# sMedX/FaceNet

Hardware: AMD Instinct MI355X
Metric: images/sec (160x160 triplet train) (higher is better)
Workload: dtype bf16

## Files before the change

facenet_amd/_lib.py:

```python
from __future__ import annotations

import ctypes as C
import os

import torch

_HERE = os.path.dirname(os.path.abspath(__file__))
LIB_PATH = os.path.join(_HERE, "lib", "libfacenet_hip.so")

FN_BF16, FN_F16 = 0, 1


class ConvDesc(C.Structure):
    _fields_ = [
        ("N", C.c_int32), ("H", C.c_int32), ("W", C.c_int32), ("Cin", C.c_int32),
        ("OH", C.c_int32), ("OW", C.c_int32), ("Cout", C.c_int32),
        ("KH", C.c_int32), ("KW", C.c_int32), ("stride", C.c_int32), ("pad_h", C.c_int32), ("pad_w", C.c_int32),
        ("dtype", C.c_int32), ("ld_x", C.c_int32), ("ld_y", C.c_int32),
        ("relu", C.c_int32), ("accumulate", C.c_int32), ("out_f32", C.c_int32), ("ld_res", C.c_int32),
        ("scale", C.c_float), ("splits", C.c_int32), ("stats_sq_off", C.c_int32), ("stats_replicas", C.c_int32),
        ("stats_rep_stride", C.c_int32),
        ("x", C.c_void_p), ("w", C.c_void_p), ("y", C.c_void_p), ("dx", C.c_void_p), ("dw", C.c_void_p),
        ("bias", C.c_void_p), ("stats", C.c_void_p), ("resid", C.c_void_p),
        ("bn_y", C.c_void_p), ("bn_scale", C.c_void_p), ("bn_shift", C.c_void_p), ("bn_beta", C.c_void_p), ("bn_acc", C.c_void_p),
        ("ld_bn_y", C.c_int32), ("bn_sq_off", C.c_int32), ("bn_replicas", C.c_int32), ("bn_rep_stride", C.c_int32), ("bn_relu", C.c_int32),
        ("nrm_stats", C.c_void_p), ("nrm_beta", C.c_void_p),
        ("nrm_sq_off", C.c_int32), ("nrm_replicas", C.c_int32), ("nrm_rep_stride", C.c_int32), ("nrm_count", C.c_int32),
        ("nrm_eps", C.c_float), ("nrm_z", C.c_void_p), ("tile_fwd", C.c_int32), ("tile_dgrad", C.c_int32),
        ("dy2", C.c_void_p), ("w2", C.c_void_p), ("dy3", C.c_void_p), ("w3", C.c_void_p),
        ("Cout2", C.c_int32), ("ld_y2", C.c_int32), ("Cout3", C.c_int32), ("ld_y3", C.c_int32),
        ("rb_prev", C.c_void_p), ("rb_out", C.c_void_p), ("rb_dtrunk", C.c_void_p), ("rb_dup", C.c_void_p), ("rb_dbias", C.c_void_p),
        ("rb_scale", C.c_float), ("rb_accumulate", C.c_int32), ("prelu", C.c_void_p),
    ]


class FacenetHipError(RuntimeError):
    pass


_i, _f, _p, _l, _u = C.c_int, C.c_float, C.c_void_p, C.c_long, C.c_uint32

_SIGNATURES = {
    "fn_abi_version": [],
    "fn_conv2d_fwd": [C.POINTER(ConvDesc), _p],
    "fn_conv2d_dgrad": [C.POINTER(ConvDesc), _p],
    "fn_conv2d_wgrad": [C.POINTER(ConvDesc), _p],
    "fn_conv2d_variant": [C.POINTER(ConvDesc), _i],
    "fn_block35_infer": [_p, _p, _i, _p, _p, _p, _p, _p, _p, _f, _i, _i, _p],
    "fn_block35_infer_warm": [_p, _p, _i, _p, _p, _p, _p, _p, _p, _f, _i, _p, C.c_int64, _i, _p],
    "fn_block17_infer": [_p, _p, _i, _p, _p, _p, _p, _p, _p, _p, _p, _p, _p, _f, _i, _i, _p],
    "fn_block17_infer_warm": [_p, _p, _i, _p, _p, _p, _p, _p, _p, _p, _p, _p, _p, _f, _i, _p, C.c_int64, _i, _p],
    "fn_conv2d_arg_bytes": [],
    "fn_conv2d_group_build": [C.POINTER(ConvDesc), _i, _i, _i, _p, _p, _p],
    "fn_conv2d_grouped": [_p, _p, _i, _i, _i, _i, _i, _i, _p],
    "fn_conv2d_wgrad_arg_bytes": [],
    "fn_conv2d_wgrad_group_build": [C.POINTER(ConvDesc), _i, _i, _p, _p, _p, _p],
    "fn_conv2d_wgrad_reduce": [_p, _i, _p],
    "fn_conv2d_wgrad_grouped": [_p, _p, _i, _i, _i, _i, _p],
    "fn_image_normalize": [_p, _p, _p, _i, _i, _i, _i, _p],
    "fn_image_normalize_f32": [_p, _p, _p, _i, _i, _i, _i, _p],
    "fn_image_resize_bilinear": [_p, _i, _p, _i, _i, _i, _i, _i, _p],
    "fn_bn_finalize": [_p, _i, _i, _p, _p, _p, _p, _p, _p, _p, _f, _f, _i, _p],
    "fn_crop_or_pad_u8": [_p, _p, _p, _p, _i, _i, _p],
    "fn_gather_images": [_p, _p, _p, _i, _i, _p],
    "fn_bn_relu_train_fwd": [_p, _i, _p, _i, _i, _i, _p, _i, _i, _i, _p, _p, _p, _p, _p, _f, _f, _i, _i, _p],
    "fn_bn_relu_train_bwd": [_p, _i, _p, _i, _i, _i, _p, _p, _p, _p, _p, _i, _i, _i, _i, _i, _i, _p],
    "fn_maxpool3x3s2_fwd": [_p, _i, _p, _i, _i, _i, _i, _i, _p, _i, _p],
    "fn_maxpool3x3s2_bwd": [_p, _i, _p, _i, _p, _i, _i, _i, _i, _i, _p, _i, _i, _p],
    "fn_area_resize_crop": [_p, _i, _i, _p, _i, _i, _i, _i, _p, _i, _p],
    "fn_maxpool2d_fwd": [_p, _i, _p, _i, _i, _i, _i, _i, _i, _i, _i, _i, _i, _i, _i, _p],
    "fn_area_resize_frame": [_p, _i, _i, _i, _i, _p, _p, _i, _p],
    "fn_mtcnn_candidates": [_p, C.c_long, _i, _f, _p, _p, _i, _i, _i, _p],
    "fn_nms_greedy_batch": [_p, _i, _p, _p, _p, _p, _i, _p, C.c_long, _p, _p, _p],
    "fn_nms_greedy": [_p, _i, _p, _i, C.c_double, _i, _p, C.c_long, _p, _p, _p],
    "fn_avgpool_fwd": [_p, _p, _i, _i, _i, _i, _p],
    "fn_avgpool_bwd": [_p, _p, _i, _i, _i, _i, _p],
    "fn_avgpool3x3s1_fwd": [_p, _i, _p, _i, _i, _i, _i, _i, _i, _p],
    "fn_avgpool3x3s1_bwd": [_p, _i, _p, _i, _i, _i, _i, _i, _i, _i, _p],
    "fn_dropout_fwd": [_p, _p, _i, _i, _f, _u, _i, _p, _i, _p],
    "fn_dropout_bwd": [_p, _p, _i, _i, _f, _u, _i, _p, _i, _p],
# ... 61 lines not shown
```

facenet_amd/csrc/conv_igemm.hip:

```cpp
#include "common.h"
#include "../../include/facenet_hip.h"
#include "wgrad_taps.h"
#include <cstdio>
#include <type_traits>
#include <cstdlib>

#ifndef FN_IG_DBG
#define FN_IG_DBG 0
#endif

#if FN_IG_DBG & 32
__device__ unsigned long long fn_ig_phase[256 * 576 * 16];
extern "C" int fn_debug_phases(unsigned long long* out, int reset) {
    static unsigned long long host[256 * 576 * 16];
    if (out) {
        if (hipMemcpyFromSymbol(host, HIP_SYMBOL(fn_ig_phase), sizeof(host)) != hipSuccess) return -1;
        for (int i = 0; i < 576 * 16; ++i) {
            out[i] = 0;
            for (int r = 0; r < 256; ++r) out[i] += host[r * 576 * 16 + i];
        }
    }
    if (reset) {
        for (auto& v : host) v = 0;
        if (hipMemcpyToSymbol(HIP_SYMBOL(fn_ig_phase), host, sizeof(host)) != hipSuccess) return -1;
// ... 22 lines not shown
    const unsigned short* resid;
    int M, PH, PW;
    int SH, SW;
    int CS;
    int NOUT, KTOT, KH, KW;
    int so, sk, offy, offx, dshift;
    int ld_src, ld_out, ld_res;
    int relu, accumulate, out_f32;
    float scale;
    int tiles_m, tiles_n;
    int stats_sq_off, stats_replicas, stats_rep_stride;
    int plain;
    const unsigned short* bn_y;
    const float* bn_scale;
    const float* bn_shift;
    const float* bn_beta;
    acc_t* bn_acc;
    int ld_bn_y, bn_sq_off, bn_replicas, bn_rep_stride, bn_relu;
    int s2;
    int cp1, cp2, cp3;
    int total_tiles;
    int src_bytes, w_bytes;
    int tile;
    int nocheck;
    const unsigned short* src2; const unsigned short* wp2;
    const unsigned short* src3; const unsigned short* wp3;
    int K2, ld2, K3, ld3, t1, t2, nt_total, src2_bytes, w2_bytes, src3_bytes, w3_bytes;
    const acc_t* nrm_stats;
    const float* nrm_beta;
    int nrm_sq_off, nrm_replicas, nrm_rep_stride, nrm_count;
    float nrm_eps;
    unsigned short* nrm_z;
    int halo_ty, halo_tx;
    const unsigned short* mask;
    unsigned short* out2;
    acc_t* colsum;
    float scale2;
    const float* prelu;
};

__device__ __forceinline__ void rcp_divmod(int m, int d, int& q, int& r) { fast_divmod(m, d, __builtin_amdgcn_rcpf((float)d), q, r); }

__device__ __forceinline__ int ktab_entry_s2(int kgroup, int CS, int KH, int KW, int qy, int qx) {
    const int nky = (KH - qy + 1) >> 1, nkx = (KW - qx + 1) >> 1;
    const int k = kgroup * 8;
    if (k >= nky * nkx * CS) return -1;
    int tap, c, ty, tx;
    rcp_divmod(k, CS, tap, c);
    rcp_divmod(tap, nkx, ty, tx);
    return ((qy + 2 * ty) << 24) | ((qx + 2 * tx) << 16) | c;
}

__device__ __forceinline__ int ktab_entry(int kgroup, int KTOT, int CS, int KW) {
    const int k = kgroup * 8;
    if (k >= KTOT) return -1;
    int tap, c, ky, kx;
    rcp_divmod(k, CS, tap, c);
    rcp_divmod(tap, KW, ky, kx);
    return (ky << 24) | (kx << 16) | c;
}

template <typename T, int BM, int BN, int WM, int WN, bool MULTI = false>
__device__ __forceinline__ void conv_epilogue(const ConvArgs& a, f32x4 (&acc)[BM / WM / 16][BN / WN / 16], unsigned char* smem, float* sRed,
                                              const int* sRow, const bool rowtab, const int m0, const int n0, const int tm, const bool active FN_EP_PARAM) {
    constexpr int TM = BM / WM, TN = BN / WN;
    constexpr int MREP = TM / 16, NREP = TN / 16;
// ... 887 lines not shown
enum { TILE_HALO = 9000000 };
static bool halo_capable(const ConvArgs& a) {
    return !a.s2 && !a.plain && a.so == 1 && a.dshift == 0 && a.KH == 3 && a.KW == 3 && a.CS % 8 == 0 && !a.nrm_stats && a.nt_total == 0;
}
static bool halo_eligible(const ConvArgs& a) {
    if (a.tile == TILE_HALO) return halo_capable(a);
    static const int enabled = getenv("FN_CONV_HALO") ? atoi(getenv("FN_CONV_HALO")) : 1;
    static const int maxc = getenv("FN_CONV_HALO_MAXC") ? atoi(getenv("FN_CONV_HALO_MAXC")) : 64;
    return enabled && halo_capable(a) && a.CS <= maxc && a.PH >= 30 && a.PW >= 30 &&
           a.tile == 0;
}
static int halo_bn(const ConvArgs& a) { return a.NOUT <= 32 ? 32 : (a.NOUT <= 48 || (a.NOUT > 64 && a.NOUT <= 96) ? 32 : 64); }

template <typename T, int BN, int WM, int WN, int KH, int KW> static int launch_halo_p(ConvArgs a, hipStream_t st) {
    a.halo_ty = cdiv(a.PH, 8);
    a.halo_tx = cdiv(a.PW, 16);
    a.tiles_n = cdiv(a.NOUT, BN);
    a.tiles_m = 0;
    const long total = (long)(a.M / (a.PH * a.PW)) * a.halo_ty * a.halo_tx * a.tiles_n;
    FN_REQUIRE(total < (1L << 24), "conv_halo: too many tiles");
    a.total_tiles = (int)total;
    const size_t smem = halo_smem_bytes(BN, KH, KW);
    auto kern = conv_halo_kernel<T, BN, WM, WN, KH, KW>;
    static LdsOptIn lds_ok;
    if (int rc = allow_big_lds(reinterpret_cast<const void*>(kern), lds_ok, "conv_halo")) return rc;
    hipLaunchKernelGGL(kern, dim3(a.total_tiles), dim3(256), smem, st, a);
    return check_launch("conv_halo");
}

template <typename T> static int launch_halo(const ConvArgs& a, hipStream_t st) {
    return halo_bn(a) == 32 ? launch_halo_p<T, 32, 4, 1, 3, 3>(a, st) : launch_halo_p<T, 64, 2, 2, 3, 3>(a, st);
}

static void plan_tiles(ConvArgs& a, int BM, int BN) {
    a.tiles_n = cdiv(a.NOUT, BN);
    if (!a.s2) {
        a.tiles_m = cdiv(a.M, BM);
        a.total_tiles = a.tiles_m * a.tiles_n;
        return;
    }
    const int nimg = a.M / (a.PH * a.PW);
    int ny[4], nx[4], pre[5];
    int t = 0;
    for (int c = 0; c < 4; ++c) {
        const int qy = c >> 1, qx = c & 1;
        const int y0 = (qy - a.offy) & 1, x0 = (qx - a.offx) & 1;
        ny[c] = a.PH > y0 ? (a.PH - y0 + 1) / 2 : 0;
        nx[c] = a.PW > x0 ? (a.PW - x0 + 1) / 2 : 0;
        pre[c] = t;
        t += cdiv(nimg * ny[c] * nx[c], BM) * a.tiles_n;
    }
    a.cp1 = pre[1]; a.cp2 = pre[2]; a.cp3 = pre[3];
    a.tiles_m = 0;
    a.total_tiles = t;
}

static size_t conv_smem_bytes(int BM, int BN, int KTOT, int plain, int norm_channels, int ks) {
    const int STAGE = ks * 2 * (BM * 128 + BN * 128);
    const int CB = BM * (BN + 4) * 4;
    return (size_t)(STAGE > CB ? STAGE : CB) + 8 * BN * 4 + (plain ? 0 : (size_t)cdiv(KTOT, 64) * 8 * 16) + (size_t)BM * 4 +
           (size_t)norm_channels * 8;
}

template <typename T, int BM, int BN, int WM, int WN, int DEPTH, int KS, bool PLAIN, int MODE>
static int launch_conv_grouped_p(const ConvArgs* dev_args, const int32_t* dev_prefix, int n, int total, size_t smem, hipStream_t st) {
    auto kern = conv_igemm_grouped_kernel<T, BM, BN, WM, WN, DEPTH, KS, PLAIN, MODE>;
// ... 20 lines not shown
}

template <typename T, int BM, int BN, int WM, int WN, int DEPTH, int KS>
static int launch_conv(const ConvArgs& a, hipStream_t st) {
    if constexpr (KS == 1) {
        if (a.nt_total > 0) return launch_conv_p<T, BM, BN, WM, WN, DEPTH, 1, true, 2>(a, st);
        if (a.nrm_stats)
            return a.plain ? launch_conv_p<T, BM, BN, WM, WN, DEPTH, 1, true, 1>(a, st) : launch_conv_p<T, BM, BN, WM, WN, DEPTH, 1, false, 1>(a, st);
    }
    return a.plain ? launch_conv_p<T, BM, BN, WM, WN, DEPTH, KS, true, 0>(a, st) : launch_conv_p<T, BM, BN, WM, WN, DEPTH, KS, false, 0>(a, st);
}

static void choose_conv_tile_auto(int M, int NOUT, int& bm, int& bn) {
    bn = 128;
    long best = (long)cdiv(NOUT, 128) * 128;
    for (int c : {64, 32}) {
        const long w = (long)cdiv(NOUT, c) * c;
        if (w < best) { best = w; bn = c; }
    }
    static const int minb = getenv("FN_CONV_MINBLOCKS") ? atoi(getenv("FN_CONV_MINBLOCKS")) : 384;
    bm = 32;
    for (int c : {128, 64}) {
        if ((long)cdiv(M, c) * cdiv(NOUT, bn) >= minb) { bm = c; break; }
    }
    while (bm == 32 && bn > 32 && (long)cdiv(M, 32) * cdiv(NOUT, bn) < minb) bn >>= 1;
}

static void choose_conv_tile(int M, int NOUT, int forced, int& bm, int& bn) {
    if (forced > 0) { bm = forced / 1000; bn = forced % 1000; return; }
    choose_conv_tile_auto(M, NOUT, bm, bn);
}

static bool valid_tile(int t) {
    if (t == 0 || t == TILE_HALO) return true;
    const int bm = t / 1000, bn = t % 1000;
    return (bm == 128 || bm == 64 || bm == 32) && (bn == 128 || bn == 64 || bn == 32);
}

static int choose_conv_ks(int M, int NOUT, int KTOT, int bm, int bn) {
    static const int force = getenv("FN_CONV_KS") ? atoi(getenv("FN_CONV_KS")) : 0;
    if (bm == 64) {
        static const int ks64 = getenv("FN_CONV_KS64") ? atoi(getenv("FN_CONV_KS64")) : 256;
        static const int ks64_4 = getenv("FN_CONV_KS64_4") ? atoi(getenv("FN_CONV_KS64_4")) : 0;
        const long grid = (long)cdiv(M, 64) * cdiv(NOUT, bn);
        if (force != 1 && force != 2 && bn <= 64 && cdiv(KTOT, 64) >= 12 && grid <= ks64_4) return 4;
        return (force != 1 && bn <= 64 && cdiv(KTOT, 64) >= 8 && grid <= ks64) ? 2 : 1;
    }
    if (bm != 32) return 1;
    const long blocks = (long)cdiv(M, 32) * cdiv(NOUT, bn);
    const int ntk = cdiv(KTOT, 64);
    static const int lim2 = getenv("FN_CONV_KS32_2") ? atoi(getenv("FN_CONV_KS32_2")) : 128;
    static const int lim4 = getenv("FN_CONV_KS32_4") ? atoi(getenv("FN_CONV_KS32_4")) : 64;
    int ks = 1;
    if (ntk >= 8 && blocks <= lim2) ks = 2;
    if (ntk >= 16 && blocks <= lim4 && bn <= 64) ks = 4;
    if (force == 1) ks = 1;
    if (force == 2 && ks > 2) ks = 2;
    return ks;
}

#define FN_CONV_VARIANTS(X) X(128, 128, 2, 2, 1, 1) X(128, 64, 2, 2, 2, 1) X(128, 32, 4, 1, 2, 1) X(64, 128, 1, 4, 2, 1) X(64, 64, 2, 2, 2, 1) \
    X(64, 32, 2, 2, 2, 1) X(32, 128, 1, 4, 4, 1) X(32, 64, 1, 4, 4, 1) X(32, 32, 2, 2, 4, 1)                                           \
    X(32, 128, 1, 4, 4, 2) X(32, 64, 1, 4, 4, 2) X(32, 64, 1, 4, 4, 4) X(32, 32, 2, 2, 4, 2) X(32, 32, 2, 2, 4, 4)                       \
    X(64, 64, 2, 2, 2, 2) X(64, 32, 2, 2, 2, 2) X(64, 64, 2, 2, 2, 4) X(64, 32, 2, 2, 2, 4)

static int variant_code(int bm, int bn, int ks) { return bm * 1000 + bn + (ks > 1 ? ks * 1000000 : 0); }

template <typename T> static int dispatch_conv(const ConvArgs& a, hipStream_t st) {
    if (halo_eligible(a)) return launch_halo<T>(a, st);
    if (a.tile == TILE_HALO) {
        set_error("conv: the halo-tile kernel was requested (tile %d) for a layer it cannot run (needs 3x3, stride 1, channels %% 8 == 0)", a.tile);
        return FN_EUNSUPPORTED;
    }
    int bm, bn;
    choose_conv_tile(a.M, a.NOUT, a.tile, bm, bn);
    if (const char* f = getenv("FN_CONV_TILE")) {
        int fm = 0, fnn = 0;
        if (sscanf(f, "%dx%d", &fm, &fnn) == 2) { bm = fm; bn = fnn; }
    }
    const int ks = (a.nrm_stats || a.nt_total > 0) ? 1 : choose_conv_ks(a.M, a.NOUT, a.KTOT, bm, bn);
#define FN_X(BM_, BN_, WM_, WN_, D_, KS_) \
    if (bm == BM_ && bn == BN_ && ks == KS_) return launch_conv<T, BM_, BN_, WM_, WN_, D_, KS_>(a, st);
    FN_CONV_VARIANTS(FN_X)
#undef FN_X
    set_error("conv: no tile variant %dx%d ks=%d", bm, bn, ks);
    return FN_EUNSUPPORTED;
}

template <typename T>
static int dispatch_conv_grouped(const ConvArgs* dev_args, const int32_t* dev_prefix, int n, int total, int bm, int bn, int ks, int plain,
                                 size_t smem, hipStream_t st) {
    const bool norm = (plain & 2) != 0;
    plain &= 1;
#define FN_X(BM_, BN_, WM_, WN_, D_, KS_)                                                                                                       \
    if (bm == BM_ && bn == BN_ && ks == KS_) {                                                                                                  \
        if constexpr (KS_ == 1) {                                                                                                               \
            if (norm)                                                                                                                           \
                return plain ? launch_conv_grouped_p<T, BM_, BN_, WM_, WN_, D_, 1, true, 1>(dev_args, dev_prefix, n, total, smem, st)         \
                             : launch_conv_grouped_p<T, BM_, BN_, WM_, WN_, D_, 1, false, 1>(dev_args, dev_prefix, n, total, smem, st);       \
        }                                                                                                                                       \
        return plain ? launch_conv_grouped_p<T, BM_, BN_, WM_, WN_, D_, KS_, true, 0>(dev_args, dev_prefix, n, total, smem, st)              \
// ... 346 lines not shown
    return bnw == 64 ? launch_wgrad<T, 128, 64>(a, splits, st) : launch_wgrad<T, 128, 128>(a, splits, st);
}

}

using namespace fn;

static int make_fwd_args(const fn_conv_desc* d, ConvArgs& a) {
    if (int rc = check_desc(d)) return rc;
    FN_REQUIRE(d->x && d->w && d->y, "conv_fwd: null x/w/y");
    FN_REQUIRE(d->ld_y >= d->Cout && (d->out_f32 ? d->ld_y % 4 == 0 : d->ld_y % 8 == 0), "conv_fwd: ld_y=%d invalid", d->ld_y);
    FN_REQUIRE(!d->resid || d->ld_res % 8 == 0, "conv_fwd: ld_res=%d invalid", d->ld_res);
    a = ConvArgs{};
    a.src = (const unsigned short*)d->x; a.wp = (const unsigned short*)d->w; a.out = d->y;
    a.bias = d->bias; a.stats = d->stats; a.resid = (const unsigned short*)d->resid;
    FN_REQUIRE(!d->prelu || (!d->resid && !d->relu && !d->accumulate && !d->stats), "conv_fwd: prelu excludes resid / relu / accumulate / stats");
    a.prelu = d->prelu;
    a.M = d->N * d->OH * d->OW; a.PH = d->OH; a.PW = d->OW; a.SH = d->H; a.SW = d->W; a.CS = d->Cin;
    a.NOUT = d->Cout; a.KTOT = d->KH * d->KW * d->Cin; a.KH = d->KH; a.KW = d->KW;
    a.so = d->stride; a.sk = 1; a.offy = -d->pad_h; a.offx = -d->pad_w; a.dshift = 0;
    a.ld_src = d->ld_x; a.ld_out = d->ld_y; a.ld_res = d->ld_res;
    a.relu = d->relu; a.accumulate = d->accumulate; a.out_f32 = d->out_f32; a.scale = d->scale;
    a.stats_sq_off = d->stats_sq_off;
    a.plain = (d->KH == 1 && d->KW == 1 && d->stride == 1 && d->pad_h == 0 && d->pad_w == 0) ? 1 : 0;
    a.nocheck = (d->pad_h == 0 && d->pad_w == 0) ? 1 : 0;
    a.stats_replicas = d->stats_replicas > 0 ? d->stats_replicas : 1;
    a.stats_rep_stride = d->stats_rep_stride;
    FN_REQUIRE((long)d->N * d->H * d->W * d->ld_x * 2 < (1L << 30) && (long)d->Cout * a.KTOT * 2 < (1L << 30),
               "conv_fwd: x or w exceeds the 1 GiB range of 32-bit buffer offsets");
    FN_REQUIRE((long)a.M * d->ld_y * (d->out_f32 ? 4 : 2) < (1L << 31) && (!d->resid || (long)a.M * d->ld_res * 2 < (1L << 31)),
               "conv_fwd: y or the residual exceeds the 2 GiB range of 32-bit byte offsets");
    a.src_bytes = d->N * d->H * d->W * d->ld_x * 2;
    a.w_bytes = d->Cout * a.KTOT * 2;
    FN_REQUIRE(valid_tile(d->tile_fwd), "conv_fwd: tile_fwd=%d is not one of {128,64,32}x{128,64,32} or 9000000 (halo)", d->tile_fwd);
    a.tile = d->tile_fwd;
    if (d->nrm_stats) {
        FN_REQUIRE(d->nrm_beta && d->Cin <= 512 && d->nrm_count > 0 && d->nrm_eps > 0.f, "conv_fwd: normalise-on-load needs beta, Cin <= 512, count, eps");
        a.nrm_stats = d->nrm_stats; a.nrm_beta = d->nrm_beta; a.nrm_sq_off = d->nrm_sq_off;
        a.nrm_replicas = d->nrm_replicas > 0 ? d->nrm_replicas : 1; a.nrm_rep_stride = d->nrm_rep_stride;
        a.nrm_count = d->nrm_count; a.nrm_eps = d->nrm_eps;
        if (d->nrm_z) {
            FN_REQUIRE(d->stride == 1 && d->OH == d->H && d->OW == d->W, "conv_fwd: nrm_z needs stride 1 and an output map of the input's size");
            a.nrm_z = (unsigned short*)d->nrm_z;
        }
    } else {
        FN_REQUIRE(!d->nrm_z, "conv_fwd: nrm_z without nrm_stats");
    }
    return FN_OK;
}

static int make_dgrad_args(const fn_conv_desc* d, ConvArgs& a) {
    if (int rc = check_desc(d)) return rc;
    FN_REQUIRE(d->y && d->w && (d->dx || d->rb_dup), "conv_dgrad: null dy/wt/dx");
    FN_REQUIRE(d->Cout % 8 == 0 && d->ld_y % 8 == 0 && d->ld_y >= d->Cout, "conv_dgrad: Cout=%d ld_y=%d must be multiples of 8", d->Cout,
               d->ld_y);
    a = ConvArgs{};
    a.src = (const unsigned short*)d->y; a.wp = (const unsigned short*)d->w; a.out = d->dx;
    a.M = d->N * d->H * d->W; a.PH = d->H; a.PW = d->W; a.SH = d->OH; a.SW = d->OW; a.CS = d->Cout;
    a.NOUT = d->Cin; a.KTOT = d->KH * d->KW * d->Cout; a.KH = d->KH; a.KW = d->KW;
    a.so = 1; a.sk = -1; a.offy = d->pad_h; a.offx = d->pad_w; a.dshift = d->stride == 2 ? 1 : 0;
    a.s2 = d->stride == 2 ? 1 : 0;
    a.ld_src = d->ld_y; a.ld_out = d->ld_x; a.ld_res = 0;
    a.relu = 0; a.accumulate = d->accumulate; a.out_f32 = d->out_f32; a.scale = 1.f;
    a.plain = (d->KH == 1 && d->KW == 1 && d->stride == 1 && d->pad_h == 0 && d->pad_w == 0) ? 1 : 0;
    a.stats_replicas = 1;
    FN_REQUIRE((long)d->N * d->OH * d->OW * d->ld_y * 2 < (1L << 30) && (long)d->Cin * a.KTOT * 2 < (1L << 30),
               "conv_dgrad: dy or wt exceeds the 1 GiB range of 32-bit buffer offsets");
    FN_REQUIRE((long)d->N * d->H * d->W * d->ld_x * (d->out_f32 ? 4 : 2) < (1L << 31) &&
                   (!d->bn_y || (long)d->N * d->H * d->W * d->ld_bn_y * 2 < (1L << 31)),
               "conv_dgrad: dx or bn_y exceeds the 2 GiB range of 32-bit byte offsets");
    a.src_bytes = d->N * d->OH * d->OW * d->ld_y * 2;
    a.w_bytes = d->Cin * a.KTOT * 2;
    FN_REQUIRE(valid_tile(d->tile_dgrad), "conv_dgrad: tile_dgrad=%d is not one of {128,64,32}x{128,64,32} or 9000000 (halo)", d->tile_dgrad);
    a.tile = d->tile_dgrad;
    if (d->dy2) {
        FN_REQUIRE(a.plain && d->w2 && d->Cout2 > 0 && d->Cout2 % 8 == 0 && d->ld_y2 % 8 == 0 && d->ld_y2 >= d->Cout2 && !d->bn_y,
                   "conv_dgrad: sibling sources need a 1x1 stride-1 layer, w2 and Cout2/ld_y2 multiples of 8");
        FN_REQUIRE(!d->dy3 || (d->w3 && d->Cout3 > 0 && d->Cout3 % 8 == 0 && d->ld_y3 % 8 == 0 && d->ld_y3 >= d->Cout3),
                   "conv_dgrad: third source needs w3 and Cout3/ld_y3 multiples of 8");
        const long pix = (long)d->N * d->OH * d->OW;
        FN_REQUIRE(pix * d->ld_y2 * 2 < (1L << 30) && (!d->dy3 || pix * d->ld_y3 * 2 < (1L << 30)), "conv_dgrad: sibling dy exceeds 1 GiB");
        a.src2 = (const unsigned short*)d->dy2; a.wp2 = (const unsigned short*)d->w2; a.K2 = d->Cout2; a.ld2 = d->ld_y2;
        a.src2_bytes = (int)(pix * d->ld_y2 * 2); a.w2_bytes = d->Cin * d->Cout2 * 2;
        a.t1 = cdiv(a.KTOT, 64);
        a.t2 = a.t1 + cdiv(a.K2, 64);
        a.nt_total = a.t2;
        if (d->dy3) {
            a.src3 = (const unsigned short*)d->dy3; a.wp3 = (const unsigned short*)d->w3; a.K3 = d->Cout3; a.ld3 = d->ld_y3;
            a.src3_bytes = (int)(pix * d->ld_y3 * 2); a.w3_bytes = d->Cin * d->Cout3 * 2;
            a.nt_total = a.t2 + cdiv(a.K3, 64);
        }
    }
    if (d->rb_dup) {
        FN_REQUIRE(d->rb_dtrunk && d->rb_dbias && !d->bn_y && !d->out_f32 && d->Cin % 8 == 0 && d->ld_x % 8 == 0,
                   "conv_dgrad: fused residual backward needs rb_dtrunk, rb_dbias, a low-precision dx geometry and no fused BN reduction");
        a.out = d->rb_dtrunk; a.accumulate = d->rb_accumulate;
        a.resid = (const unsigned short*)d->rb_prev; a.ld_res = d->ld_x; a.scale = 1.f;
        a.mask = (const unsigned short*)d->rb_out; a.out2 = (unsigned short*)d->rb_dup; a.colsum = d->rb_dbias; a.scale2 = d->rb_scale;
    }
    if (d->bn_y) {
        FN_REQUIRE(!d->accumulate && !d->out_f32 && d->bn_scale && d->bn_shift && d->bn_beta && d->bn_acc && d->ld_bn_y % 8 == 0,
                   "conv_dgrad: fused BN reduction needs a sole-writer low-precision dx and all bn_* pointers");
        a.bn_y = (const unsigned short*)d->bn_y; a.bn_scale = d->bn_scale; a.bn_shift = d->bn_shift; a.bn_beta = d->bn_beta;
        a.bn_acc = d->bn_acc; a.ld_bn_y = d->ld_bn_y; a.bn_sq_off = d->bn_sq_off;
        a.bn_replicas = d->bn_replicas > 0 ? d->bn_replicas : 1; a.bn_rep_stride = d->bn_rep_stride; a.bn_relu = d->bn_relu;
    }
// ... 154 lines not shown
}

template <typename T> static int launch_wgrad_grouped(const void* args, const int32_t* prefix, int n, int total, int variant, hipStream_t st) {
    const bool norm = variant >= 1000000;
    variant %= 1000000;
    const int bmw = variant / 1000, bnw = variant % 1000;
    const unsigned char* a = reinterpret_cast<const unsigned char*>(args);
    const int stride_ = fn_conv2d_wgrad_arg_bytes();
#define FN_WG(BM_, BN_)                                                                                                     \
    if (bmw == BM_ && bnw == BN_) {                                                                                         \
        const size_t sm_ = 2 * 64 * ((BM_) * 2 + 32 + (BN_) * 2 + 32) + (norm ? 2 * (BN_) * 4 : 0);                            \
        if (norm) hipLaunchKernelGGL((conv_wgrad_grouped_kernel<T, BM_, BN_, true>), dim3(total), dim3(256), sm_, st, a, stride_, prefix, n); \
        else hipLaunchKernelGGL((conv_wgrad_grouped_kernel<T, BM_, BN_, false>), dim3(total), dim3(256), sm_, st, a, stride_, prefix, n);    \
        return check_launch("conv_wgrad_grouped");                                                                          \
    }
    FN_WG(32, 64) FN_WG(32, 128) FN_WG(64, 64) FN_WG(64, 128) FN_WG(128, 64) FN_WG(128, 128)
#undef FN_WG
    set_error("wgrad_grouped: unknown variant %d", variant);
    return FN_EINVAL;
}

extern "C" int fn_conv2d_wgrad_grouped(const void* dev_args, const int32_t* dev_prefix, int n, int total_blocks, int variant, int dtype,
                                       void* stream) {
    FN_REQUIRE(dev_args && dev_prefix && n > 0 && total_blocks > 0, "wgrad_grouped: bad arguments");
    FN_REQUIRE(dtype == FN_BF16 || dtype == FN_F16, "dtype %d unsupported", dtype);
    if (variant >= WGRAD_TAPS_VARIANT) return wgrad_taps_launch(dev_args, dev_prefix, n, total_blocks, variant, dtype, (hipStream_t)stream);
    return dtype == FN_BF16 ? launch_wgrad_grouped<__bf16>(dev_args, dev_prefix, n, total_blocks, variant, (hipStream_t)stream)
                            : launch_wgrad_grouped<_Float16>(dev_args, dev_prefix, n, total_blocks, variant, (hipStream_t)stream);
}

extern "C" int fn_conv2d_variant(const fn_conv_desc* d, int op) {
    if (!d || op < 0 || op > 2) return FN_EINVAL;
    int a, b;
    if (op < 2) {
        ConvArgs ca;
        if ((op == 0 ? make_fwd_args(d, ca) : make_dgrad_args(d, ca)) == FN_OK && halo_eligible(ca)) return 9000000 + halo_bn(ca);
        if ((op == 0 ? d->tile_fwd : d->tile_dgrad) == TILE_HALO) return FN_EUNSUPPORTED;
    }
    if (op == 0) {
        choose_conv_tile(d->N * d->OH * d->OW, d->Cout, valid_tile(d->tile_fwd) ? d->tile_fwd : 0, a, b);
        return variant_code(a, b, d->nrm_stats ? 1 : choose_conv_ks(d->N * d->OH * d->OW, d->Cout, d->KH * d->KW * d->Cin, a, b));
    }
    if (op == 1) {
        choose_conv_tile(d->N * d->H * d->W, d->Cin, valid_tile(d->tile_dgrad) ? d->tile_dgrad : 0, a, b);
        return variant_code(a, b, d->dy2 ? 1 : choose_conv_ks(d->N * d->H * d->W, d->Cin, d->KH * d->KW * d->Cout, a, b));
    }
    if (const int tv = wgrad_taps_variant(d)) return tv;
    final_wgrad_tile(d->Cout, d->KH * d->KW * d->Cin, a, b);
    return a * 1000 + b;
}
```

facenet_amd/train.py:

```python
from __future__ import annotations

import ctypes as C
import json
import os
from typing import Callable, Dict, List, Optional, Sequence, Tuple

import numpy as np
import torch

from . import _lib, parallel
from .engine import BN_EPS, L2_WEIGHT, Lowering, Network, _pad8, _ptr
from .schedule import Op, Schedule, StreamSet, levelize, make_events, region, run_schedule, torch_op


class GraphRunner:

    def __init__(self, device: torch.device):
        self.device = device
        self.graphs: List[torch.cuda.CUDAGraph] = []
        self.pool = None

    def capture(self, fn: Callable[[], None]) -> torch.cuda.CUDAGraph:
        g = torch.cuda.CUDAGraph()
        with torch.cuda.graph(g, pool=self.pool):
# ... 27 lines not shown
        total = lib.fn_conv2d_wgrad_group_build(descs, n, variant, host_args, host_prefix, None, C.byref(ws_elems))
        if total < 0:
            _lib.check(total, "wgrad_group_build")
        ws = torch.empty(max(1, ws_elems.value), dtype=torch.float32, device=net.device)
        total = lib.fn_conv2d_wgrad_group_build(descs, n, variant, host_args, host_prefix, _ptr(ws), C.byref(ws_elems))
        if total < 0:
            _lib.check(total, "wgrad_group_build")
        dev_args = torch.frombuffer(bytearray(host_args), dtype=torch.uint8).to(net.device)
        dev_prefix = torch.tensor(list(host_prefix), dtype=torch.int32, device=net.device)
        reads, writes = [], []
        for m in members:
            reads.extend(m.reads)
            writes.extend(m.writes)
        if variant >= 5000000:
            code = variant - 5000000
            name = f"conv_wgrad_taps:{code // 1000}x{code % 1000 // 10}" + ("s2" if code % 10 else "")
        else:
            name = f"conv_wgrad_grouped:{variant % 1000000 // 1000}x{variant % 1000}" + (":norm" if variant >= 1000000 else "")
        out.append(Op(name, lib.fn_conv2d_wgrad_grouped,
                      (_ptr(dev_args), _ptr(dev_prefix), n, total, variant, dt), keep=(descs, dev_args, dev_prefix, members, ws),
                      reads=tuple(reads), writes=tuple(writes) + (region(ws),)))
        if ws_elems.value > 0:
            split_tables.append(dev_args)
            split_keep.append(ws)
            split_writes.extend(writes)
    if split_tables:
        table = torch.cat(split_tables)
        out.append(Op("conv_wgrad_reduce", lib.fn_conv2d_wgrad_reduce, (_ptr(table), table.numel() // nbytes), keep=(table, split_keep),
                      reads=tuple(region(w) for w in split_keep), writes=tuple(split_writes)))
    return out


TILE_CANDIDATES = tuple((bm, bn) for bm in (128, 64, 32) for bn in (128, 64, 32))


def autotune_convs(ops: Sequence[Op], net: Network, launches: int = 8, rounds: int = 2) -> Dict[str, int]:
    if os.environ.get("FACENET_AUTOTUNE", "1") == "0":
        return {}
    lib, st = net.lib, net.stream()
    chosen: Dict[str, int] = {}
    cache_path = os.environ.get("FACENET_TUNE_CACHE")
    cache: Dict[str, int] = {}
    if cache_path and os.path.exists(cache_path):
        with open(cache_path) as fh:
            cache = json.load(fh)
    dirty = False

    def burst(op):
        a, b = torch.cuda.Event(enable_timing=True), torch.cuda.Event(enable_timing=True)
        a.record()
        for _ in range(launches):
            rc = op.fn(*op.args, st)
            if rc:
                return float("inf")
        b.record()
        b.synchronize()
        return a.elapsed_time(b)

    for op in ops:
        kind = op.name.split(":")[0]
        if kind not in ("conv_fwd", "conv_dgrad") or not op.keep or not isinstance(op.keep[0], _lib.ConvDesc):
            continue
        d = op.keep[0]
        field = "tile_fwd" if kind == "conv_fwd" else "tile_dgrad"
        nout = d.Cout if kind == "conv_fwd" else d.Cin
        key = f"{op.name}|N{d.N}|{d.H}x{d.W}x{d.Cin}|dt{d.dtype}|nrm{int(bool(d.nrm_stats))}"
        if key in cache:
            setattr(d, field, int(cache[key]))
            chosen[op.name] = int(cache[key])
            continue
        setattr(d, field, 0)
        base_code = lib.fn_conv2d_variant(C.byref(d), 0 if kind == "conv_fwd" else 1)
        base = base_code % 1000000
        timings = {}
        if base_code >= 9000000:
            base = 0
            burst(op)
            timings[0] = min(burst(op) for _ in range(rounds))
        for bm, bn in TILE_CANDIDATES:
            if bn > 32 and bn // 2 >= nout:
                continue
            setattr(d, field, bm * 1000 + bn)
            burst(op)
            timings[bm * 1000 + bn] = min(burst(op) for _ in range(rounds))
        best = min(timings, key=timings.get)
        if base in timings and timings[best] > 0.97 * timings[base]:
            best = base
        setattr(d, field, best)
        chosen[op.name] = best
        cache[key] = best
        dirty = True
    torch.cuda.synchronize()
    if cache_path and dirty:
        tmp = f"{cache_path}.{os.getpid()}.tmp"
        with open(tmp, "w") as fh:
            json.dump(cache, fh, indent=0)
        os.replace(tmp, cache_path)
    return chosen


def group_convs(ops: List[Op], net: Network) -> List[Op]:
    lib = net.lib
    level = levelize(ops)
    order = sorted(range(len(ops)), key=lambda i: (level[i], i))
    nbytes = lib.fn_conv2d_arg_bytes()
    buckets = {}
    for i in order:
        op = ops[i]
        kind = op.name.split(":")[0]
        if kind in ("conv_fwd", "conv_dgrad") and op.keep and isinstance(op.keep[0], _lib.ConvDesc) and not op.keep[0].dy2:
            d = op.keep[0]
            opi = 0 if kind == "conv_fwd" else 1
            if lib.fn_conv2d_variant(C.byref(d), opi) >= 9000000:
                continue
            plain = int(d.KH == 1 and d.KW == 1 and d.stride == 1 and d.pad_h == 0 and d.pad_w == 0)
            if opi == 0 and d.nrm_stats:
                plain |= 2
# ... 510 lines not shown
```

include/facenet_hip.h:

```cpp
#ifndef FACENET_HIP_H
#define FACENET_HIP_H
#include <stdint.h>
#ifdef __cplusplus
extern "C" {
#endif

#define FN_BF16 0
#define FN_F16 1

typedef int64_t fn_acc_t;
#define FN_ACC_STAT_BITS 20
#define FN_ACC_GRAD_BITS 40

const char* fn_last_error(void);
int fn_abi_version(void);

typedef struct fn_conv_desc {
    int32_t N, H, W, Cin;
    int32_t OH, OW, Cout;
    int32_t KH, KW, stride, pad_h, pad_w;
    int32_t dtype;
    int32_t ld_x, ld_y;
    int32_t relu;
    int32_t accumulate;
// ... 33 lines not shown
    const void* rb_out;
    void* rb_dtrunk;
    void* rb_dup;
    fn_acc_t* rb_dbias;
    float rb_scale;
    int32_t rb_accumulate;
    const float* prelu;
} fn_conv_desc;

int fn_block17_infer(const void* x, void* y, int N, const void* w_t0, const void* w_t1a, const void* w_t1b, const void* w_t1c, const void* w_up,
                     const float* b_t0, const float* b_t1a, const float* b_t1b, const float* b_t1c, const float* b_up, float scale, int relu,
                     int dtype, void* stream);
int fn_block17_infer_warm(const void* x, void* y, int N, const void* w_t0, const void* w_t1a, const void* w_t1b, const void* w_t1c,
                          const void* w_up, const float* b_t0, const float* b_t1a, const float* b_t1b, const float* b_t1c, const float* b_up,
                          float scale, int relu, const void* warm, int64_t warm_bytes, int dtype, void* stream);
int fn_block35_infer(const void* x, void* y, int N, const void* const* w_1x1, const void* const* w_3x3, const void* w_up,
                     const float* const* b_1x1, const float* const* b_3x3, const float* b_up, float scale, int relu, int dtype, void* stream);
int fn_block35_infer_warm(const void* x, void* y, int N, const void* const* w_1x1, const void* const* w_3x3, const void* w_up,
                          const float* const* b_1x1, const float* const* b_3x3, const float* b_up, float scale, int relu,
                          const void* warm, int64_t warm_bytes, int dtype, void* stream);
int fn_conv2d_fwd(const fn_conv_desc* d, void* stream);
int fn_conv2d_dgrad(const fn_conv_desc* d, void* stream);
int fn_conv2d_wgrad(const fn_conv_desc* d, void* stream);
int fn_conv2d_arg_bytes(void);
int fn_conv2d_group_build(const fn_conv_desc* descs, int n, int op, int variant, void* host_args, int32_t* host_prefix, int32_t* smem_bytes);
int fn_conv2d_grouped(const void* dev_args, const int32_t* dev_prefix, int n, int total_blocks, int variant, int plain, int smem_bytes,
                      int dtype, void* stream);
int fn_conv2d_wgrad_arg_bytes(void);
int fn_conv2d_wgrad_group_build(const fn_conv_desc* descs, int n, int variant, void* host_args, int32_t* host_prefix, float* ws,
                                int64_t* ws_elems);
int fn_conv2d_wgrad_grouped(const void* dev_args, const int32_t* dev_prefix, int n, int total_blocks, int variant, int dtype, void* stream);
int fn_conv2d_wgrad_reduce(const void* dev_args, int n, void* stream);
int fn_conv2d_variant(const fn_conv_desc* d, int op);

int fn_image_normalize(const uint8_t* img, void* out, float* work, int N, int HW, int mode, int dtype, void* stream);
int fn_image_normalize_f32(const float* img, void* out, float* work, int N, int HW, int mode, int dtype, void* stream);
int fn_image_resize_bilinear(const void* img, int src_is_f32, float* out, int N, int H, int W, int OH, int OW, void* stream);
int fn_crop_or_pad_u8(const uint8_t* src, const long long* offsets, const int32_t* hw, uint8_t* dst, int N, int S, void* stream);
int fn_gather_images(const uint8_t* pool, const int32_t* idx, uint8_t* out, int n_out, int bytes_per_image, void* stream);

int fn_bn_finalize(const fn_acc_t* stats, int sq_off, int rep_stride, const int32_t* reps, const int32_t* count, const float* beta,
                   float* save_scale, float* save_shift, float* moving_mean, float* moving_var, float momentum, float eps, int CB,
                   void* stream);

int fn_bn_relu_train_fwd(const void* y, int ld_y, void* z, int ld_z, int M, int C, const fn_acc_t* stats, int stats_sq_off, int stats_replicas,
                         int stats_rep_stride, const float* beta,
                         float* save_scale, float* save_shift, float* moving_mean, float* moving_var, float momentum, float eps,
                         int relu, int dtype, void* stream);
int fn_bn_relu_train_bwd(void* dz, int ld_d, const void* y, int ld_y, int M, int C, const float* beta, const float* save_scale,
                         const float* save_shift, float* dbeta, fn_acc_t* acc, int acc_sq_off, int acc_replicas, int acc_rep_stride,
                         int reduced, int relu, int dtype, void* stream);

int fn_maxpool3x3s2_fwd(const void* x, int ld_x, void* y, int ld_y, int N, int H, int W, int C, uint8_t* argmax, int dtype, void* stream);
int fn_maxpool3x3s2_bwd(const void* x, int ld_x, const void* dy, int ld_dy, void* dx, int ld_dx, int N, int H, int W, int C,
                        const uint8_t* argmax, int accumulate, int dtype, void* stream);
int fn_area_resize_crop(const uint8_t* frame, int H, int W, const int32_t* boxes, int n, int OH, int OW, int source_is_u8, void* out,
                        int dtype, void* stream);
int fn_maxpool2d_fwd(const void* x, int ld_x, void* y, int ld_y, int N, int H, int W, int C, int k, int stride, int pad_h, int pad_w,
                     int OH, int OW, int dtype, void* stream);
int fn_area_resize_frame(const uint8_t* frame, int H, int W, int OH, int OW, float* rows, void* out, int dtype, void* stream);
int fn_mtcnn_candidates(const float* map, long ncell, int ld, float threshold, float* cand, int32_t* counter, int max_cand, int tag,
                        int reset_counter, void* stream);
int fn_nms_greedy(const double* boxes, int ld, const int32_t* order, int n, double threshold, int by_min, void* workspace,
                  long workspace_bytes, int32_t* keep, int32_t* n_keep, void* stream);
int fn_nms_greedy_batch(const double* boxes, int ld, const int32_t* order, const int32_t* sizes, const double* thresholds, const int32_t* by_min,
                        int njobs, void* workspace, long workspace_bytes, int32_t* keep, int32_t* n_keep, void* stream);
// ... 49 lines not shown
```

Baseline: 13900.

## Add patch-tap 3x3 conv kernel with row-tile LDS patch reuse and autotune it

Adds a new implicit-GEMM kernel for 3x3 stride-1 convolutions (forward and dgrad). Each block loads a multi-row input patch with halo into LDS once per channel slice and reuses it across all nine taps, with double-buffered patch and weight rings. The autotuner now times this variant per layer and keeps it only when it beats the baseline by a margin. It costs a lot of LDS per block (up to 160 KiB), which can lower occupancy, and leaves some waste in partially filled row tiles.

```diff
diff --git a/facenet_amd/_lib.py b/facenet_amd/_lib.py
--- a/facenet_amd/_lib.py
+++ b/facenet_amd/_lib.py
@@ -46,6 +46,7 @@
     "fn_conv2d_dgrad": [C.POINTER(ConvDesc), _p],
     "fn_conv2d_wgrad": [C.POINTER(ConvDesc), _p],
     "fn_conv2d_variant": [C.POINTER(ConvDesc), _i],
+    "fn_conv2d_patch_plan": [_i, _i, _i, _p],
     "fn_block35_infer": [_p, _p, _i, _p, _p, _p, _p, _p, _p, _f, _i, _i, _p],
     "fn_block35_infer_warm": [_p, _p, _i, _p, _p, _p, _p, _p, _p, _f, _i, _p, C.c_int64, _i, _p],
     "fn_block17_infer": [_p, _p, _i, _p, _p, _p, _p, _p, _p, _p, _p, _p, _p, _f, _i, _i, _p],
diff --git a/facenet_amd/csrc/conv_igemm.hip b/facenet_amd/csrc/conv_igemm.hip
--- a/facenet_amd/csrc/conv_igemm.hip
+++ b/facenet_amd/csrc/conv_igemm.hip
@@ -78,6 +78,8 @@
     float nrm_eps;
     unsigned short* nrm_z;
     int halo_ty, halo_tx;
+    int pt_rows, pt_blocks;
+    int pt_rs, pt_plane;
     const unsigned short* mask;
     unsigned short* out2;
     acc_t* colsum;
@@ -1031,6 +1033,261 @@
     return halo_bn(a) == 32 ? launch_halo_p<T, 32, 4, 1, 3, 3>(a, st) : launch_halo_p<T, 64, 2, 2, 3, 3>(a, st);
 }
 
+enum { TILE_PATCH = 9100000 };
+constexpr int patch_npl(int mrep) { return mrep == 5 ? 6 : 8; }
+
+template <int BN> struct PatchRing {
+    static constexpr int STEP = 3 * BN;
+    static constexpr int PLANE = STEP * 32 + 64;
+    static constexpr int BUF = 2 * PLANE;
+};
+
+template <typename T, int BN, int MREP>
+__global__ __launch_bounds__(256, 2) void conv_patch_kernel(const ConvArgs a) {
+    constexpr int WM = 4, BM = 64 * MREP, TM = BM / WM, NREP = BN / 16;
+    constexpr int NWL = (PatchRing<BN>::STEP * 4 + 255) / 256, PATCH_NPL = patch_npl(MREP);
+    constexpr int WPLANE = PatchRing<BN>::PLANE, WBUF = PatchRing<BN>::BUF;
+    constexpr int CPART = 128 * (BN + 4) * 4;
+    typedef typename LP<T>::vec8 vec8;
+
+    extern __shared__ __attribute__((aligned(16))) unsigned char smem[];
+    const int RS = a.pt_rs, PPLANE = a.pt_plane, PBUF = 2 * PPLANE;
+    unsigned char* sW = smem + 2 * PBUF;
+    const int stage = 2 * PBUF + 2 * WBUF;
+    float* sRed = reinterpret_cast<float*>(smem + (stage > CPART ? stage : CPART));
+    int* sRow = reinterpret_cast<int*>(sRed + 8 * BN);
+
+    const int tid = threadIdx.x, lane = tid & 63, wave = tid >> 6;
+    const int fr = lane & 15, fq = lane >> 4;
+    const int R = a.pt_rows, PW = a.PW, PWt = PW + 2, NPIX = (R + 2) * PWt;
+    int sp, tn, n, rb;
+    rcp_divmod(xcd_remap(blockIdx.x, a.total_tiles), a.tiles_n, sp, tn);
+    rcp_divmod(sp, a.pt_blocks, n, rb);
+    const int oy0 = rb * R, n0 = tn * BN;
+    const int nvalid = min(R, a.PH - oy0) * PW;
+    const bool fwd = a.sk > 0;
+    const int sy0 = oy0 + a.offy - (fwd ? 0 : 2), sx0 = a.offx - (fwd ? 0 : 2);
+
+    for (int e = tid; e < BM; e += 256) {
+        const int h0 = (e >> 7) * 2, hn = MREP - h0 < 2 ? MREP - h0 : 2, r = e - 64 * h0;
+        const int w = r / (16 * hn), i = h0 + (r >> 4) % hn;
+        const int s = w * TM + i * 16 + (r & 15);
+        int q = -1;
+        if (s < nvalid) {
+            int yy, xx;
+            rcp_divmod(s, PW, yy, xx);
+            q = (n * a.PH + oy0 + yy) * PW + xx;
+        }
+        sRow[e] = q;
+    }
+
+    constexpr unsigned OOB = 0x60000000u;
+    const __amdgpu_buffer_rsrc_t rs_src = __builtin_amdgcn_make_buffer_rsrc(const_cast<unsigned short*>(a.src), 0, a.src_bytes, 0x00020000);
+    const __amdgpu_buffer_rsrc_t rs_w = __builtin_amdgcn_make_buffer_rsrc(const_cast<unsigned short*>(a.wp), 0, a.w_bytes, 0x00020000);
+    unsigned poff[PATCH_NPL], woff[NWL];
+    int plds[PATCH_NPL], wlds[NWL];
+#pragma unroll
+    for (int i = 0; i < PATCH_NPL; ++i) {
+        const int idx = tid + 256 * i, p = idx >> 2, ch = idx & 3;
+        int pr, pc;
+        rcp_divmod(p, PWt, pr, pc);
+        const int sy = sy0 + pr, sx = sx0 + pc;
+        const bool ok = p < NPIX && (unsigned)sy < (unsigned)a.SH && (unsigned)sx < (unsigned)a.SW;
+        poff[i] = ok ? (unsigned)(((n * a.SH + sy) * a.SW + sx) * a.ld_src + ch * 8) * 2u : OOB;
+        plds[i] = p < NPIX ? (ch >> 1) * PPLANE + pr * RS + pc * 32 + (ch & 1) * 16 : -1;
+    }
+#pragma unroll
+    for (int j = 0; j < NWL; ++j) {
+        const int idx = tid + 256 * j, rw = idx >> 2, ch = idx & 3;
+        const int px = rw / BN, co = rw % BN;
+        const bool ok = rw < PatchRing<BN>::STEP && n0 + co < a.NOUT;
+        woff[j] = ok ? (unsigned)((n0 + co) * a.KTOT + (fwd ? px : 2 - px) * a.CS + ch * 8) * 2u : OOB;
+        wlds[j] = rw < PatchRing<BN>::STEP ? (ch >> 1) * WPLANE + rw * 32 + (ch & 1) * 16 : -1;
+    }
+    int abase[MREP];
+#pragma unroll
+    for (int i = 0; i < MREP; ++i) {
+        const int s = wave * TM + i * 16 + fr;
+        int yy = 0, xx = 0;
+        if (s < nvalid) rcp_divmod(s, PW, yy, xx);
+        abase[i] = yy * RS + xx * 32 + (fq >> 1) * PPLANE + (fq & 1) * 16;
+    }
+    const int wl = (fq >> 1) * WPLANE + fr * 32 + (fq & 1) * 16;
+
+    const int nslices = (a.CS + 31) >> 5;
+    u32x4 rp[PATCH_NPL], rw_[NWL];
+    auto load_patch = [&](const int sl) {
+        const int c0 = sl * 32;
+#pragma unroll
+        for (int i = 0; i < PATCH_NPL; ++i) {
+            const int ch = (tid + 256 * i) & 3;
+            const unsigned off = (sl < nslices && c0 + ch * 8 < a.CS) ? poff[i] + (unsigned)c0 * 2u : OOB;
+            rp[i] = __builtin_amdgcn_raw_buffer_load_b128(rs_src, (int)off, 0, 0);
+        }
+    };
+    auto load_w = [&](const int sl, const int py) {
+        const int c0 = sl * 32;
+        const unsigned tb = (unsigned)(((fwd ? py : 2 - py) * 3 * a.CS + c0) * 2);
+#pragma unroll
+        for (int j = 0; j < NWL; ++j) {
+            const int ch = (tid + 256 * j) & 3;
+            const unsigned off = (sl < nslices && c0 + ch * 8 < a.CS) ? woff[j] + tb : OOB;
+            rw_[j] = __builtin_amdgcn_raw_buffer_load_b128(rs_w, (int)off, 0, 0);
+        }
+    };
+    auto store_patch = [&](const int b) {
+#pragma unroll
+        for (int i = 0; i < PATCH_NPL; ++i)
+            if (plds[i] >= 0) *reinterpret_cast<u32x4*>(smem + b * PBUF + plds[i]) = rp[i];
+    };
+    auto store_w = [&](const int wb) {
+#pragma unroll
+        for (int j = 0; j < NWL; ++j)
+            if (wlds[j] >= 0) *reinterpret_cast<u32x4*>(sW + wb * WBUF + wlds[j]) = rw_[j];
+    };
+
+    f32x4 acc[MREP][NREP];
+#pragma unroll
+    for (int i = 0; i < MREP; ++i)
+#pragma unroll
+        for (int j = 0; j < NREP; ++j) acc[i][j] = f32x4{0.f, 0.f, 0.f, 0.f};
+
+    auto step = [&](auto B, auto PY, auto WB, const int sl) {
+        constexpr int b = decltype(B)::value, py = decltype(PY)::value, wb = decltype(WB)::value;
+        if constexpr (py < 2) load_w(sl, py + 1); else load_w(sl + 1, 0);
+        if constexpr (py == 0) load_patch(sl + 1);
+        int so = b * PBUF + py * RS;
+        asm volatile("" : "+s"(so));
+        int ab[MREP];
+#pragma unroll
+        for (int i = 0; i < MREP; ++i) ab[i] = abase[i] + so;
+#pragma unroll
+        for (int px = 0; px < 3; ++px) {
+            vec8 fa[MREP], fb[NREP];
+#pragma unroll
+            for (int i = 0; i < MREP; ++i) fa[i] = *reinterpret_cast<const vec8*>(smem + ab[i] + px * 32);
+#pragma unroll
+            for (int j = 0; j < NREP; ++j) fb[j] = *reinterpret_cast<const vec8*>(sW + wb * WBUF + (px * BN + j * 16) * 32 + wl);
+#pragma unroll
+            for (int i = 0; i < MREP; ++i)
+#pragma unroll
+                for (int j = 0; j < NREP; ++j) acc[i][j] = LP<T>::mfma(fa[i], fb[j], acc[i][j]);
+        }
+        if constexpr (py == 2) store_patch(1 - b);
+        store_w(1 - wb);
+        __syncthreads();
+    };
+    using I0 = std::integral_constant<int, 0>;
+    using I1 = std::integral_constant<int, 1>;
+    using I2 = std::integral_constant<int, 2>;
+
+    load_w(0, 0);
+    load_patch(0);
+    store_w(0);
+    store_patch(0);
+    __syncthreads();
+    for (int sl = 0; sl < nslices; sl += 2) {
+        step(I0{}, I0{}, I0{}, sl);
+        step(I0{}, I1{}, I1{}, sl);
+        step(I0{}, I2{}, I0{}, sl);
+        if (sl + 1 < nslices) {
+            step(I1{}, I0{}, I1{}, sl + 1);
+            step(I1{}, I1{}, I0{}, sl + 1);
+            step(I1{}, I2{}, I1{}, sl + 1);
+        }
+    }
+#pragma unroll
+    for (int i = 0; i < MREP; ++i)
+#pragma unroll
+        for (int r = 0; r < 4; ++r) {
+            const bool ok = wave * TM + i * 16 + fq * 4 + r < nvalid;
+#pragma unroll
+            for (int j = 0; j < NREP; ++j) acc[i][j][r] = ok ? acc[i][j][r] : 0.f;
+        }
+#if FN_IG_DBG & 32
+    unsigned long long ep[4];
+#endif
+    auto part = [&](auto H0, auto HN) {
+        constexpr int h0 = decltype(H0)::value, hn = decltype(HN)::value;
+        f32x4 pa[hn][NREP];
+#pragma unroll
+        for (int i = 0; i < hn; ++i)
+#pragma unroll
+            for (int j = 0; j < NREP; ++j) pa[i][j] = acc[h0 + i][j];
+        conv_epilogue<T, 64 * hn, BN, WM, 1>(a, pa, smem, sRed, sRow + 64 * h0, true, 0, n0, sp, true FN_EP_ARG);
+    };
+    part(I0{}, std::integral_constant<int, 2>{});
+    __syncthreads();
+    if constexpr (MREP >= 4) part(I2{}, std::integral_constant<int, 2>{});
+    if constexpr (MREP == 5) {
+        __syncthreads();
+        part(std::integral_constant<int, 4>{}, I1{});
+    }
+}
+
+static int patch_bn(const ConvArgs& a) { return a.NOUT <= 32 || (a.NOUT > 64 && a.NOUT <= 96) ? 32 : 64; }
+
+static size_t patch_smem_bytes(int mrep, int bn, int R, int PW, int& rs, int& plane) {
+    rs = PW * 32 + 256;
+    plane = (R + 2) * rs;
+    plane += ((64 - plane % 128) % 128 + 128) % 128;
+    const int wbuf = bn == 32 ? PatchRing<32>::BUF : PatchRing<64>::BUF;
+    const int stage = 4 * plane + 2 * wbuf, cpart = 128 * (bn + 4) * 4;
+    return (size_t)(stage > cpart ? stage : cpart) + 8 * bn * 4 + 64 * mrep * 4;
+}
+
+static bool patch_plan(int PH, int PW, int bn, int& mrep, int& R, size_t& smem) {
+    long best = -1;
+    for (int m : {4, 5}) {
+        const int bm = 64 * m;
+        if (PW > bm) continue;
+        const int r = PH < bm / PW ? PH : bm / PW;
+        if ((r + 2) * (PW + 2) > patch_npl(m) * 64) continue;
+        int rs, plane;
+        const size_t s = patch_smem_bytes(m, bn, r, PW, rs, plane);
+        if (s > 160 * 1024) continue;
+        const long waste = (long)cdiv(PH, r) * bm - (long)PH * PW;
+        const long score = (s > 80 * 1024 ? 1L << 40 : 0) + waste;
+        if (best < 0 || score < best) { best = score; mrep = m; R = r; smem = s; }
+    }
+    return best >= 0;
+}
+
+static bool patch_capable(const ConvArgs& a) {
+    int m, r;
+    size_t s;
+    return halo_capable(a) && patch_plan(a.PH, a.PW, patch_bn(a), m, r, s);
+}
+
+template <typename T, int BN, int MREP> static int launch_patch_p(ConvArgs a, int R, size_t smem, hipStream_t st) {
+    a.pt_rows = R;
+    a.pt_blocks = cdiv(a.PH, R);
+    patch_smem_bytes(MREP, BN, R, a.PW, a.pt_rs, a.pt_plane);
+    a.tiles_n = cdiv(a.NOUT, BN);
+    a.tiles_m = 0;
+    const long total = (long)(a.M / (a.PH * a.PW)) * a.pt_blocks * a.tiles_n;
+    FN_REQUIRE(total < (1L << 24), "conv_patch: too many tiles");
+    a.total_tiles = (int)total;
+    auto kern = conv_patch_kernel<T, BN, MREP>;
+    static LdsOptIn lds_ok;
+    if (int rc = allow_big_lds(reinterpret_cast<const void*>(kern), lds_ok, "conv_patch")) return rc;
+    hipLaunchKernelGGL(kern, dim3(a.total_tiles), dim3(256), smem, st, a);
+    return check_launch("conv_patch");
+}
+
+template <typename T> static int launch_patch(const ConvArgs& a, hipStream_t st) {
+    const int bn = patch_bn(a);
+    int mrep, R;
+    size_t smem;
+    if (!halo_capable(a) || !patch_plan(a.PH, a.PW, bn, mrep, R, smem)) {
+        set_error("conv: the patch-tap kernel was requested (tile %d) for a layer it cannot run (needs 3x3, stride 1, channels %% 8 == 0, "
+                  "a row tile of at most 320 slots and a patch of at most %d pixels)", a.tile, patch_npl(4) * 64);
+        return FN_EUNSUPPORTED;
+    }
+    if (bn == 32) return mrep == 4 ? launch_patch_p<T, 32, 4>(a, R, smem, st) : launch_patch_p<T, 32, 5>(a, R, smem, st);
+    return mrep == 4 ? launch_patch_p<T, 64, 4>(a, R, smem, st) : launch_patch_p<T, 64, 5>(a, R, smem, st);
+}
+
 static void plan_tiles(ConvArgs& a, int BM, int BN) {
     a.tiles_n = cdiv(a.NOUT, BN);
     if (!a.s2) {
@@ -1117,7 +1374,7 @@
 }
 
 static bool valid_tile(int t) {
-    if (t == 0 || t == TILE_HALO) return true;
+    if (t == 0 || t == TILE_HALO || t == TILE_PATCH) return true;
     const int bm = t / 1000, bn = t % 1000;
     return (bm == 128 || bm == 64 || bm == 32) && (bn == 128 || bn == 64 || bn == 32);
 }
@@ -1152,6 +1409,7 @@
 static int variant_code(int bm, int bn, int ks) { return bm * 1000 + bn + (ks > 1 ? ks * 1000000 : 0); }
 
 template <typename T> static int dispatch_conv(const ConvArgs& a, hipStream_t st) {
+    if (a.tile == TILE_PATCH) return launch_patch<T>(a, st);
     if (halo_eligible(a)) return launch_halo<T>(a, st);
     if (a.tile == TILE_HALO) {
         set_error("conv: the halo-tile kernel was requested (tile %d) for a layer it cannot run (needs 3x3, stride 1, channels %% 8 == 0)", a.tile);
@@ -1564,7 +1822,7 @@
                "conv_fwd: y or the residual exceeds the 2 GiB range of 32-bit byte offsets");
     a.src_bytes = d->N * d->H * d->W * d->ld_x * 2;
     a.w_bytes = d->Cout * a.KTOT * 2;
-    FN_REQUIRE(valid_tile(d->tile_fwd), "conv_fwd: tile_fwd=%d is not one of {128,64,32}x{128,64,32} or 9000000 (halo)", d->tile_fwd);
+    FN_REQUIRE(valid_tile(d->tile_fwd), "conv_fwd: tile_fwd=%d is not one of {128,64,32}x{128,64,32}, 9000000 (halo) or 9100000 (patch)", d->tile_fwd);
     a.tile = d->tile_fwd;
     if (d->nrm_stats) {
         FN_REQUIRE(d->nrm_beta && d->Cin <= 512 && d->nrm_count > 0 && d->nrm_eps > 0.f, "conv_fwd: normalise-on-load needs beta, Cin <= 512, count, eps");
@@ -1603,7 +1861,7 @@
                "conv_dgrad: dx or bn_y exceeds the 2 GiB range of 32-bit byte offsets");
     a.src_bytes = d->N * d->OH * d->OW * d->ld_y * 2;
     a.w_bytes = d->Cin * a.KTOT * 2;
-    FN_REQUIRE(valid_tile(d->tile_dgrad), "conv_dgrad: tile_dgrad=%d is not one of {128,64,32}x{128,64,32} or 9000000 (halo)", d->tile_dgrad);
+    FN_REQUIRE(valid_tile(d->tile_dgrad), "conv_dgrad: tile_dgrad=%d is not one of {128,64,32}x{128,64,32}, 9000000 (halo) or 9100000 (patch)", d->tile_dgrad);
     a.tile = d->tile_dgrad;
     if (d->dy2) {
         FN_REQUIRE(a.plain && d->w2 && d->Cout2 > 0 && d->Cout2 % 8 == 0 && d->ld_y2 % 8 == 0 && d->ld_y2 >= d->Cout2 && !d->bn_y,
@@ -1824,6 +2082,11 @@
 extern "C" int fn_conv2d_variant(const fn_conv_desc* d, int op) {
     if (!d || op < 0 || op > 2) return FN_EINVAL;
     int a, b;
+    if (op < 2 && (op == 0 ? d->tile_fwd : d->tile_dgrad) == TILE_PATCH) {
+        ConvArgs ca;
+        if ((op == 0 ? make_fwd_args(d, ca) : make_dgrad_args(d, ca)) == FN_OK && patch_capable(ca)) return TILE_PATCH + patch_bn(ca);
+        return FN_EUNSUPPORTED;
+    }
     if (op < 2) {
         ConvArgs ca;
         if ((op == 0 ? make_fwd_args(d, ca) : make_dgrad_args(d, ca)) == FN_OK && halo_eligible(ca)) return 9000000 + halo_bn(ca);
@@ -1841,3 +2104,19 @@
     final_wgrad_tile(d->Cout, d->KH * d->KW * d->Cin, a, b);
     return a * 1000 + b;
 }
+
+extern "C" int fn_conv2d_patch_plan(int PH, int PW, int nout, int32_t* out) {
+    FN_REQUIRE(out && PH > 0 && PW > 0 && nout > 0, "conv_patch_plan: bad arguments");
+    ConvArgs a{};
+    a.NOUT = nout;
+    const int bn = patch_bn(a);
+    int mrep, R;
+    size_t smem;
+    if (!patch_plan(PH, PW, bn, mrep, R, smem)) {
+        set_error("conv_patch_plan: no tile of at most 320 slots, %d patch pixels and 160 KiB of LDS covers %d x %d", patch_npl(4) * 64, PH, PW);
+        return FN_EUNSUPPORTED;
+    }
+    const int blocks = cdiv(PH, R);
+    out[0] = R; out[1] = 64 * mrep; out[2] = blocks; out[3] = blocks * 64 * mrep - PH * PW; out[4] = (int32_t)smem; out[5] = bn;
+    return FN_OK;
+}
diff --git a/facenet_amd/train.py b/facenet_amd/train.py
--- a/facenet_amd/train.py
+++ b/facenet_amd/train.py
@@ -83,6 +83,7 @@
 
 
 TILE_CANDIDATES = tuple((bm, bn) for bm in (128, 64, 32) for bn in (128, 64, 32))
+TILE_PATCH = 9100000
 
 
 def autotune_convs(ops: Sequence[Op], net: Network, launches: int = 8, rounds: int = 2) -> Dict[str, int]:
@@ -134,6 +135,10 @@
             setattr(d, field, bm * 1000 + bn)
             burst(op)
             timings[bm * 1000 + bn] = min(burst(op) for _ in range(rounds))
+        setattr(d, field, TILE_PATCH)
+        if lib.fn_conv2d_variant(C.byref(d), 0 if kind == "conv_fwd" else 1) >= TILE_PATCH:
+            burst(op)
+            timings[TILE_PATCH] = min(burst(op) for _ in range(rounds))
         best = min(timings, key=timings.get)
         if base in timings and timings[best] > 0.97 * timings[base]:
             best = base
diff --git a/include/facenet_hip.h b/include/facenet_hip.h
--- a/include/facenet_hip.h
+++ b/include/facenet_hip.h
@@ -89,6 +89,7 @@
 int fn_conv2d_wgrad_grouped(const void* dev_args, const int32_t* dev_prefix, int n, int total_blocks, int variant, int dtype, void* stream);
 int fn_conv2d_wgrad_reduce(const void* dev_args, int n, void* stream);
 int fn_conv2d_variant(const fn_conv_desc* d, int op);
+int fn_conv2d_patch_plan(int PH, int PW, int nout, int32_t* out);
 
 int fn_image_normalize(const uint8_t* img, void* out, float* work, int N, int HW, int mode, int dtype, void* stream);
 int fn_image_normalize_f32(const float* img, void* out, float* work, int N, int HW, int mode, int dtype, void* stream);
```

Result: no change. 13930 (median of 6 runs) (+0.2%).
